# YHY138/Boosting-Fine-grained-Feature-Fusion-in-3D-Point-Cloud-Registration

Measured on AMD Instinct MI355X. Metric: point-cloud pairs/sec (forward) on ModelNet 2048-pt pairs, higher is better.
Workload: dtype f32 (emulated on the fp16 MFMA pipe: f16x3 split products); 1 GPU; ModelNet40 2048-pt pairs, 8 pairs per GPU (BASELINE configs[1] at N=1, configs[3] at N=8); pairs_per_gpu=8, global_batch=8, points_per_cloud=717, parallelism=pair-sharded dp1, precision=fp32

## Files before the change

boosting-fine-grained-feature-fusion-in-3d-point-cloud-registration_amd/csrc/ffn.hip:

```cpp
#include <algorithm>
#include <cstdlib>

#include "mfma.h"

namespace fgr {
namespace {

constexpr int kFfnD = 256;
constexpr int kFfnKS = kFfnD / 32;
constexpr int kFfnNP = kFfnD / 16;
constexpr int kFfnMaxF = 2048;
constexpr int kUnit = 1024;
constexpr int kRing = 8;
static_assert(kFfnKS * 128 == kUnit, "a W1 panel is one ring unit");
static_assert(kFfnNP / 2 * 128 == kUnit, "half of a chunk's W2 slice is one ring unit");

struct FfnArgs {
    const float* x; int64_t ldx;
    const float* ln_g; const float* ln_b; float eps;
    const u32x4* w1; const float* wsc1; const float* b1;
    const u32x4* w2; const float* wsc2; const float* b2;
    const float* bound;
    float* out; int64_t ldo;
    int M, F;
};

__device__ __forceinline__ void wait_units(int n) {
    static_assert(kRing - 2 <= 6, "extend the switch");
    switch (n) {
        case 0: wait_vm_lgkm0<0>(); break;
        case 1: wait_vm_lgkm0<4>(); break;
        case 2: wait_vm_lgkm0<8>(); break;
        case 3: wait_vm_lgkm0<12>(); break;
        case 4: wait_vm_lgkm0<16>(); break;
        case 5: wait_vm_lgkm0<20>(); break;
        default: wait_vm_lgkm0<24>(); break;
    }
}

typedef __attribute__((address_space(3))) u32x4 lds_u4;

__shared__ u32x4 g_ffn_ring0[kUnit], g_ffn_ring1[kUnit], g_ffn_ring2[kUnit], g_ffn_ring3[kUnit],
                 g_ffn_ring4[kUnit], g_ffn_ring5[kUnit], g_ffn_ring6[kUnit], g_ffn_ring7[kUnit];
static_assert(kRing == 8, "one object per slot below");

__device__ __forceinline__ u32x4* ring_slot(int s) {
    switch (s & 7) {
// ... 261 lines not shown
}

__device__ __forceinline__ float gelu_scaled(float sz, float isq) {
    const float a = sz * isq, t = fabsf(a), s = a * a;
    float r = fmaf(-1.72853470e-5f, t, 3.83197126e-4f);
    const float u = fmaf(-3.88396438e-3f, t, 2.42546219e-2f);
    r = fmaf(r, s, u);
    r = fmaf(r, t, -1.06777877e-1f);
    r = fmaf(r, t, -6.34846687e-1f);
    r = fmaf(r, t, -1.28717512e-1f);
    r = fmaf(r, t, -t);
    const float e = 0.5f * __expf(r);
    const float tail = a < 0.f ? e : 1.f - e;
    float q = -5.96761703e-4f;
    q = fmaf(q, s, 4.99119423e-3f);
    q = fmaf(q, s, -2.67681349e-2f);
    q = fmaf(q, s, 1.12819925e-1f);
    q = fmaf(q, s, -3.76125336e-1f);
    q = fmaf(q, s, 1.28379166e-1f);
    const float mid = fmaf(0.5f, fmaf(q, a, a), 0.5f);
    return sz * (t > 0.927734375f ? tail : mid);
}

template <int RT, int ACT = FGR_ACT_RELU>
__global__ void __launch_bounds__(256, 1) ffn_nsplit_kernel(FfnArgs p) {
    static_assert(RT >= 1 && RT <= 4, "row tiles");
    static_assert(ACT == FGR_ACT_RELU || ACT == FGR_ACT_GELU, "activation");
    __shared__ u32x4 act[RT * kFfnKS * 2 * 64];
    __shared__ u32x4 hbuf[2][4][RT][2][64];
    __shared__ float4 cw1[kFfnMaxF / 4], cb1[kFfnMaxF / 4];
    __shared__ float4 cw2[kFfnD / 4], cb2[kFfnD / 4];
    __shared__ float4 lng[kFfnD / 4], lnb[kFfnD / 4];
    __shared__ float2 rowpar[64];

    constexpr int BR = 16 * RT;
    const int nbm = (p.M + BR - 1) / BR;
    int t = blockIdx.x;
    {
        const int q = nbm / 8, r = nbm % 8, x = t % 8, lo = t / 8;
        t = (x < r ? x * (q + 1) : r * (q + 1) + (x - r) * q) + lo;
    }
    const int tid = threadIdx.x, wv = tid >> 6, lane = tid & 63;
    const int g = lane >> 4, c = lane & 15;
    const int r0 = t * BR;
    const int nst = p.F / 128;

    const int nf4 = p.F / 4;
    const int j0 = min(tid, nf4 - 1), j1 = min(tid + 256, nf4 - 1);
    const float4 pw1a = reinterpret_cast<const float4*>(p.wsc1)[j0];
    const float4 pb1a = reinterpret_cast<const float4*>(p.b1)[j0];
    const float4 pw1b = reinterpret_cast<const float4*>(p.wsc1)[j1];
    const float4 pb1b = reinterpret_cast<const float4*>(p.b1)[j1];
    const int t4 = tid & (kFfnD / 4 - 1);
    const float4 pw2 = reinterpret_cast<const float4*>(p.wsc2)[t4];
    const float4 pb2 = reinterpret_cast<const float4*>(p.b2)[t4];
    const float4 pg = reinterpret_cast<const float4*>(p.ln_g)[t4];
    const float4 pbe = reinterpret_cast<const float4*>(p.ln_b)[t4];
    __builtin_amdgcn_sched_barrier(0);
    float xr[kFfnKS][8];
    {
        const int64_t row = min(r0 + 16 * min(wv, RT - 1) + c, p.M - 1);
        const float* ar = p.x + row * p.ldx;
#pragma unroll
        for (int s = 0; s < kFfnKS; ++s) {
            const float4 a0 = *reinterpret_cast<const float4*>(ar + 32 * s + 8 * g);
            const float4 a1 = *reinterpret_cast<const float4*>(ar + 32 * s + 8 * g + 4);
            xr[s][0] = a0.x; xr[s][1] = a0.y; xr[s][2] = a0.z; xr[s][3] = a0.w;
            xr[s][4] = a1.x; xr[s][5] = a1.y; xr[s][6] = a1.z; xr[s][7] = a1.w;
        }
    }
    {
        if (tid < nf4) { cw1[tid] = pw1a; cb1[tid] = pb1a; }
        if (tid + 256 < nf4) { cw1[tid + 256] = pw1b; cb1[tid + 256] = pb1b; }
        if (tid < kFfnD / 4) { cw2[tid] = pw2; cb2[tid] = pb2; lng[tid] = pg; lnb[tid] = pbe; }
    }
    const float bM1 = p.bound[0], bMb = p.bound[1];
    __syncthreads();

    {
        float sm = 0.f;
#pragma unroll
        for (int s = 0; s < kFfnKS; ++s)
            sm += ((xr[s][0] + xr[s][1]) + (xr[s][2] + xr[s][3])) +
                  ((xr[s][4] + xr[s][5]) + (xr[s][6] + xr[s][7]));
        const float mean = xg_sum(sm) / (float)kFfnD;
        float sq = 0.f;
#pragma unroll
        for (int s = 0; s < kFfnKS; ++s)
#pragma unroll
            for (int e = 0; e < 8; ++e) {
                const float d = xr[s][e] - mean;
                sq += d * d;
            }
        const float rstd = 1.0f / sqrtf(xg_sum(sq) / (float)kFfnD + p.eps);
        float mx = 0.f, nn = 0.f;
#pragma unroll
        for (int s = 0; s < kFfnKS; ++s) {
            const int k = 32 * s + 8 * g;
            const float4 g0 = lng[k / 4], g1 = lng[k / 4 + 1];
            const float4 b0 = lnb[k / 4], b1 = lnb[k / 4 + 1];
            const float gg[8] = {g0.x, g0.y, g0.z, g0.w, g1.x, g1.y, g1.z, g1.w};
            const float bb[8] = {b0.x, b0.y, b0.z, b0.w, b1.x, b1.y, b1.z, b1.w};
// ... 150 lines not shown
                        const f16x8 wh = __builtin_bit_cast(f16x8, wf[2 * qq]);
                        const f16x8 wl = __builtin_bit_cast(f16x8, wf[2 * qq + 1]);
                        f32x4& a = accy[rt][2 * qh + qq];
                        a = __builtin_amdgcn_mfma_f32_16x16x32_f16(wl, hh, a, 0, 0, 0);
                        a = __builtin_amdgcn_mfma_f32_16x16x32_f16(wh, hl, a, 0, 0, 0);
                        a = __builtin_amdgcn_mfma_f32_16x16x32_f16(wh, hh, a, 0, 0, 0);
                    }
                }
                __builtin_amdgcn_sched_group_barrier(0x008, 6 * RT, 0);
                __builtin_amdgcn_sched_barrier(0);
            }
        }
    }
    wait_vm_only(0);

#pragma unroll
    for (int rt = 0; rt < RT; ++rt) {
        const int rr = r0 + 16 * rt + c;
        const int64_t row = min(rr, p.M - 1);
        const float inv_s = 1.f / rowpar[16 * rt + c].y;
        const float* xrow = p.x + row * p.ldx;
        float4 res[4];
#pragma unroll
        for (int q = 0; q < 4; ++q) res[q] = *reinterpret_cast<const float4*>(xrow + 16 * (4 * wv + q) + 4 * g);
        float* orow = p.out + row * p.ldo;
#pragma unroll
        for (int q = 0; q < 4; ++q) {
            const int n = 16 * (4 * wv + q) + 4 * g;
            const float4 w4 = cw2[n / 4], b4 = cb2[n / 4];
            const float4 y = make_float4(fmaf(accy[rt][q][0], w4.x * inv_s, b4.x) + res[q].x,
                                         fmaf(accy[rt][q][1], w4.y * inv_s, b4.y) + res[q].y,
                                         fmaf(accy[rt][q][2], w4.z * inv_s, b4.z) + res[q].z,
                                         fmaf(accy[rt][q][3], w4.w * inv_s, b4.w) + res[q].w);
            if (rr < p.M) *reinterpret_cast<float4*>(orow + n) = y;
        }
    }
}

__global__ void __launch_bounds__(256)
ffn_w2_split_kernel(const float* __restrict__ w, int n, int f, int64_t sn, int64_t sk,
                    float* __restrict__ wsc, u32x4* __restrict__ img) {
    const int tid = threadIdx.x, q = blockIdx.x, r0 = q * 16;
    const int ri = tid >> 4, kl = tid & 15;
    float mx = 0.f;
    if (r0 + ri < n)
        for (int j = kl; j < f; j += 16) mx = fmaxf(mx, fabsf(w[(int64_t)(r0 + ri) * sn + (int64_t)j * sk]));
    __shared__ float red[16][17];
    __shared__ float scale_inv[16];
    red[ri][kl] = mx;
    __syncthreads();
    if (tid < 16) {
        float m = 0.f;
#pragma unroll
        for (int z = 0; z < 16; ++z) m = fmaxf(m, red[tid][z]);
        const int e = row_scale_exp(m);
        const bool ok = r0 + tid < n;
        scale_inv[tid] = ok ? __builtin_ldexpf(1.f, e) : 0.f;
// ... 86 lines not shown
    if (m == 0) return FGR_OK;
    hipStream_t st = as_stream(stream);
    TimedCall timed_(st);
    const char* i1 = static_cast<const char*>(w1_img);
    const char* i2 = static_cast<const char*>(w2_img);
    FfnArgs a{x, ldx, gamma, beta, eps,
              (const u32x4*)i1, (const float*)(i1 + (size_t)(f / 16) * kFfnKS * 128 * 16), b1,
              (const u32x4*)i2, (const float*)(i2 + ffn_image_bytes(d, f)), b2,
              bound, out, ldo, m, f};
    const bool rt3 = (m + 47) / 48 <= kCusFfn && (m + 63) / 64 < kCusFfn;
    if (act == FGR_ACT_GELU) {
        const unsigned nb = (unsigned)((m + 47) / 48);
        hipLaunchKernelGGL((ffn_nsplit_kernel<3, FGR_ACT_GELU>), dim3(nb), dim3(256), 0, st, a);
    } else if (f % 128 == 0) {
        if (rt3)
            hipLaunchKernelGGL(ffn_nsplit_kernel<3>, dim3((unsigned)((m + 47) / 48)), dim3(256), 0, st, a);
        else
            hipLaunchKernelGGL(ffn_nsplit_kernel<4>, dim3((unsigned)((m + 63) / 64)), dim3(256), 0, st, a);
    } else
        hipLaunchKernelGGL(ffn_f16x3_kernel, dim3((unsigned)((m + 63) / 64)), dim3(256), 0, st, a);
    FGR_CHECK_LAUNCH("ffn_f16x3_kernel");
    return FGR_OK;
}
```

boosting-fine-grained-feature-fusion-in-3d-point-cloud-registration_amd/fgreg/_lib.py:

```python
import ctypes
import os
import subprocess

HERE = os.path.dirname(os.path.abspath(__file__))
LIB_PATH = os.environ.get('FGREG_LIB_PATH') or os.path.join(HERE, 'libfgreg.so')
CSRC = os.path.join(os.path.dirname(HERE), 'csrc')

_vp = ctypes.c_void_p
_i32 = ctypes.c_int32
_i64 = ctypes.c_int64
_f32 = ctypes.c_float
_sz = ctypes.c_size_t

ABI_VERSION = 2

SIGNATURES = {
    'fgr_grid_subsample_workspace': [_i64, _i32, _i64, ctypes.POINTER(_sz)],
    'fgr_grid_subsample_count': [_vp, _vp, _i32, _i64, _f32, _i64, _vp, _sz, _vp, _vp],
    'fgr_grid_subsample_fill': [_i64, _i32, _i64, _i64, _vp, _sz, _vp, _vp, _vp, _vp],
    'fgr_grid_subsample_sparse_workspace': [_i64, _i32, ctypes.POINTER(_sz)],
    'fgr_grid_subsample_sparse_count': [_vp, _vp, _i32, _i64, _f32, _i32, _vp, _sz, _vp, _vp],
    'fgr_grid_subsample_sparse_fill': [_i64, _i32, _i64, _vp, _sz, _vp, _vp, _vp, _vp],
    'fgr_radius_grid_workspace': [_i64, _i32, ctypes.POINTER(_sz)],
    'fgr_radius_grid_build': [_vp, _vp, _i32, _i64, _f32, _vp, _sz, _vp],
# ... 36 lines not shown
                                  ctypes.c_uint32, _f32, _vp, _vp],
    'fgr_attention_bf16_workspace': [_i64, _i32, _i32, ctypes.POINTER(_sz)],
    'fgr_attention_bf16': [_vp, _i64, _vp, _i64, _vp, _i64, _vp, _i64, _vp, _vp, _vp, _i32, _i32,
                           _i64, _i32, _i32, _i32, _i32, _f32, _vp, _i64, _vp],
    'fgr_res2net_chain6': [_vp, _i64, _i32, _i32, _vp, _vp, _vp, _i32, _vp, _i64, _vp],
    'fgr_res2net_chain_h3': [_vp, _i64, _i32, _i32, _vp, _vp, _vp, _vp, _i32, _vp, _i64, _vp],
    'fgr_res2net_block_h3': [_vp, _i64, _i32, _i32, _i32, _vp, _vp, _vp, _vp, _vp, _vp, _vp, _i64,
                             _vp],
    'fgr_res2net_block6': [_vp, _i64, _i32, _i32, _i32, _vp, _vp, _vp, _vp, _vp, _vp, _i64, _vp],
    'fgr_split_weights_h3_bytes': [_i32, _i32, ctypes.POINTER(_sz)],
    'fgr_split_weights_h3_batch': [_vp, _i32, _i64, _vp],
    'fgr_split_weights_h3': [_vp, _i32, _i32, _i64, _i64, _vp, _vp],
    'fgr_gemm_f16x3': [_vp, _i64, _vp, _vp, _i64, _vp, _vp, _i64, _i32, _i32, _i32, _i32, _vp],
    'fgr_gemm_f16x3_ln_supported': [_i32, _i32, _i32],
    'fgr_gemm_f16x3_ln': [_vp, _i64, _vp, _vp, _f32, _vp, _i64, _vp, _vp, _i64, _vp, _i32, _i32,
                          _i32, _i32, _vp],
    'fgr_gemm_f16x3_ln_out2': [_vp, _i64, _vp, _vp, _f32, _vp, _i64, _vp, _vp, _i64, _vp, _i32,
                               _i32, _i32, _i32, _vp, _vp, _vp, _i64, _vp],
    'fgr_split_weights_ffn2_bytes': [_i32, _i32, ctypes.POINTER(_sz)],
    'fgr_split_weights_ffn2': [_vp, _i32, _i32, _i64, _i64, _vp, _vp],
    'fgr_ffn_f16x3_supported': [_i32, _i32, _i32],
    'fgr_ffn_f16x3': [_vp, _i64, _vp, _vp, _f32, _vp, _vp, _vp, _vp, _vp, _vp, _i64, _i32, _i32,
                      _i32, _vp],
    'fgr_ffn_f16x3_act_supported': [_i32, _i32, _i32, _i32],
    'fgr_ffn_f16x3_act': [_vp, _i64, _vp, _vp, _f32, _vp, _vp, _vp, _vp, _vp, _vp, _i64, _i32,
                          _i32, _i32, _i32, _vp],
    'fgr_gelu_fwd': [_vp, _vp, _i64, _vp],
    'fgr_gelu_bwd': [_vp, _vp, _vp, _i64, _vp],
    'fgr_pos_mlp_f16x3_supported': [_i64, _i32],
    'fgr_pos_mlp_f16x3': [_vp, _i64, _vp, _vp, _vp, _vp, _vp, _vp, _vp, _vp, _vp, _vp, _i32, _vp,
                          _i64, _vp],
    'fgr_split_weights_bf16_bytes': [_i32, _i32, ctypes.POINTER(_sz)],
    'fgr_split_weights_bf16': [_vp, _i32, _i32, _i64, _i64, _vp, _vp],
    'fgr_gemm_bf16': [_vp, _i64, _vp, _vp, _i64, _vp, _vp, _i64, _i32, _i32, _i32, _i32, _vp],
    'fgr_gemm_workspace': [_i32, _i32, _i32, _i32, ctypes.POINTER(_sz)],
    'fgr_gemm_f16x3_ws': [_vp, _i64, _vp, _vp, _i64, _vp, _vp, _i64, _i32, _i32, _i32, _i32, _vp,
                          _sz, _vp],
    'fgr_gemm_bf16_ws': [_vp, _i64, _vp, _vp, _i64, _vp, _vp, _i64, _i32, _i32, _i32, _i32, _vp,
                         _sz, _vp],
    'fgr_kv_image_bytes': [_i64, _i32, _i32, ctypes.POINTER(_sz)],
    'fgr_gemm_f16x3_ln_qkv_supported': [_i32, _i32, _i32],
    'fgr_gemm_f16x3_ln_qkv': [_vp, _i64, _vp, _vp, _f32, _vp, _i64, _vp, _vp, _i64, _vp, _i32, _i32,
                              _i32, _vp, _vp, _vp, _vp, _i64, _vp],
    'fgr_gemm_f16x3_qkv_supported': [_i32, _i32, _i32],
    'fgr_gemm_f16x3_qkv': [_vp, _i64, _vp, _vp, _i64, _vp, _i32, _i32, _i32, _vp, _vp],
    'fgr_kv_image_bf16_bytes': [_i64, _i32, _i32, ctypes.POINTER(_sz)],
# ... 135 lines not shown
```

boosting-fine-grained-feature-fusion-in-3d-point-cloud-registration_amd/fgreg/ops.py:

```python
import ctypes
import math
from typing import Optional, Sequence, Tuple

import torch

from . import _lib
from ._lib import (ACT_GELU, ACT_LEAKY, ACT_NONE, ACT_RELU, ACT_RELU_RES_LEAKY,
                   NB_DIST, NB_INDEX)


def _ptr(t):
    return None if t is None else t.data_ptr()


class KernelTimer:

    def __init__(self, names):
        self.names = set(names)
        self.events = {n: [] for n in names}
        self.work = {n: [] for n in names}
        self.labels = {n: [] for n in names}
        self.count = False
        self.pool = []
        self.lead_cycles = 0
# ... 818 lines not shown
    t0 = _begin('gemm', (n, 3 * d, d))
    gemm_fn = 'fgr_gemm_f16x3_qkv' if mode == 'f16x3' else 'fgr_gemm_bf16_qkv'
    _lib.check(getattr(L, gemm_fn)(_ptr(h), h.stride(0), _ptr(w_img.img), _ptr(q), q.stride(0),
                                   _ptr(bias), n, d, n_head, _ptr(img), _stream()), gemm_fn)
    _end('gemm', t0, 2 * n * 3 * d * d)
    o = torch.empty((n, d), dtype=torch.float32, device=h.device)
    t0 = _begin('attention')
    attn_fn = 'fgr_attention_f16x3_img' if mode == 'f16x3' else 'fgr_attention_bf16_img'
    _lib.check(getattr(L, attn_fn)(
        _ptr(q), q.stride(0), _ptr(img), n, _ptr(o), o.stride(0), _ptr(q_off), _ptr(q_off),
        _ptr(kv_seg), q_off.numel() - 1, int(max_len), n_head, d // n_head,
        float(math.sqrt(1.0 / float(d // n_head))), _stream()), attn_fn)
    _end('attention', t0, lambda: attention_flops(q_off, q_off, kv_seg, d))
    return o


FFN_FUSE = True


def ffn_supported(m, d, f, act=ACT_RELU) -> bool:
    return FFN_FUSE and bool(_lib.load().fgr_ffn_f16x3_act_supported(m, d, f, act))


def ffn(x, norm, w1_img, b1, w2_img, b2, bound, out=None, act=ACT_RELU) -> torch.Tensor:
    _dev(x, b1, b2, bound)
    m, d = x.shape
    f = b1.numel()
    assert x.dtype == torch.float32 and x.stride(1) == 1 and b2.numel() == d
    x = x if (x.stride(0) % 4 == 0 and x.data_ptr() % 16 == 0) else x.contiguous()
    g, b = norm.weight.contiguous(), norm.bias.contiguous()
    b1, b2, bound = b1.contiguous(), b2.contiguous(), bound.contiguous()
    if out is None:
        out = torch.empty((m, d), dtype=torch.float32, device=x.device)
    t0 = _begin('gemm', ('ffn', m, d, f))
    _lib.check(_lib.load().fgr_ffn_f16x3_act(
        _ptr(x), x.stride(0), _ptr(g), _ptr(b), float(norm.eps), _ptr(w1_img.img), _ptr(b1),
        _ptr(w2_img.img), _ptr(b2), _ptr(bound), _ptr(out), out.stride(0), m, d, f, int(act),
        _stream()), 'fgr_ffn_f16x3_act')
    _end('gemm', t0, 4 * m * d * f)
    return out


def gelu(z, out=None) -> torch.Tensor:
    _dev(z, out)
    assert z.dtype == torch.float32 and z.is_contiguous()
    if out is None:
        out = torch.empty_like(z)
    assert out.dtype == torch.float32 and out.is_contiguous() and out.shape == z.shape
    _lib.check(_lib.load().fgr_gelu_fwd(_ptr(z), _ptr(out), z.numel(), _stream()), 'fgr_gelu_fwd')
    return out


def gelu_(z) -> torch.Tensor:
    return gelu(z, out=z)


def gelu_backward(z, dy, out=None) -> torch.Tensor:
    _dev(z, dy, out)
    assert z.dtype == torch.float32 and z.is_contiguous()
    dy = _c(dy, torch.float32)
    assert dy.shape == z.shape
    if out is None:
# ... 119 lines not shown
```

boosting-fine-grained-feature-fusion-in-3d-point-cloud-registration_amd/fgreg/transformer.py:

```python
import copy

import torch
import torch.nn as nn

from . import linear as lin
from . import ops
from .linear import linear, linear_ln, ln_fusable

class Segments:

    def __init__(self, lengths, device, n_layers=0, phantoms=None):
        self.lengths = [int(n) for n in lengths]
        n = len(self.lengths)
        assert n % 2 == 0
        self.B = n // 2
        self.phantoms = [int(p) for p in phantoms] if phantoms is not None else [0] * n
        assert len(self.phantoms) == n and min(self.phantoms, default=0) >= 0
        self.seg_cloud = list(range(n)) + [c for c in range(n) if self.phantoms[c] > 0]
        self.seg_lengths = self.lengths + [p for p in self.phantoms if p > 0]
        self.n_phantom = sum(self.phantoms)
        self.off = ops.offsets(self.seg_lengths, device)
        self.cloud_off = self.off[:n + 1]
        self.self_seg = ops.to_device(self.seg_cloud, torch.int32, device)
        self.cross_seg = ops.to_device([(c + self.B) % n for c in self.seg_cloud], torch.int32,
# ... 66 lines not shown
                and ops.qkv_bf16_supported(h_pos.shape[0], d, self.nhead)):
            return ops.qkv_attention(h_pos, lin.weight_image(W, mode='bf16'), b, seg.off, kv_seg,
                                     seg.max_len, self.nhead, mode='bf16')
        if val_has_pos:
            qkv = linear(h_pos, W, b)
            q, k, v = qkv[:, :d], qkv[:, d:2 * d], qkv[:, 2 * d:]
        else:
            qk = linear(h_pos, W, b[:2 * d], rows=(0, 2 * d))
            q, k = qk[:, :d], qk[:, d:]
            v = linear(h_nopos, W, b[2 * d:], rows=(2 * d, 3 * d))
        o = ops.attention(q, k, v, seg.off, seg.off, kv_seg, seg.max_len, self.nhead)
        return o

    def takes_side(self, x, pos):
        n, d = x.shape
        return (self.normalize_before and self.sa_val_has_pos_emb and pos is not None
                and ln_fusable(n, 3 * d, d))

    def wants_h1(self, x):
        n, d = x.shape
        return (self.normalize_before and self.sa_val_has_pos_emb
                and not ln_fusable(n, 3 * d, d))

    def forward_packed(self, x, pos, seg: Segments, pending_bias=None, h1=None, side=None):
        if not self.normalize_before:
            return self._forward_post(x, pos, seg, pending_bias), None
        n, d = x.shape
        fuse_in = ln_fusable(n, 3 * d, d)
        if fuse_in and self.sa_val_has_pos_emb and pending_bias is None:
            o = self._attend(self.self_attn, None, None, True, seg, seg.self_seg,
                             ln=(x, self.norm1, pos), side=side)
            side = None
        elif h1 is not None:
            assert pending_bias is None and self.sa_val_has_pos_emb
            o = self._attend(self.self_attn, h1, None, True, seg, seg.self_seg)
        else:
            if side is not None:
                ops.layernorm(x, side[0].weight, side[0].bias, side[0].eps, out=side[1])
                side = None
            h = ops.layernorm(x, self.norm1.weight, self.norm1.bias, self.norm1.eps, add=pos,
                              pre_bias=pending_bias)
            h0 = None if self.sa_val_has_pos_emb else ops.layernorm(
                x, self.norm1.weight, self.norm1.bias, self.norm1.eps)
            o = self._attend(self.self_attn, h, h0, self.sa_val_has_pos_emb, seg, seg.self_seg)
        x = linear(o, self.self_attn.out_proj.weight, self.self_attn.out_proj.bias, residual=x)
        if fuse_in and self.ca_val_has_pos_emb:
            o = self._attend(self.multihead_attn, None, None, True, seg, seg.cross_seg,
                             ln=(x, self.norm2, pos))
        else:
            h = ops.layernorm(x, self.norm2.weight, self.norm2.bias, self.norm2.eps, add=pos)
            h0 = None if self.ca_val_has_pos_emb else ops.layernorm(
                x, self.norm2.weight, self.norm2.bias, self.norm2.eps)
            o = self._attend(self.multihead_attn, h, h0, self.ca_val_has_pos_emb, seg,
                             seg.cross_seg)
        x = linear(o, self.multihead_attn.out_proj.weight, self.multihead_attn.out_proj.bias,
                   residual=x)
        if lin.MODE == 'f16x3' and ops.ffn_supported(n, d, self.linear1.out_features, self.act):
            return ops.ffn(x, self.norm3, lin.weight_image(self.linear1.weight, mode='f16x3'),
                           self.linear1.bias, lin.weight_image(self.linear2.weight, mode='ffn2'),
                           self.linear2.bias, self._ffn_bound(), act=self.act), None
        if self.act == ops.ACT_GELU:
            h = ops.gelu_(linear_ln(x, self.norm3, self.linear1.weight, self.linear1.bias))
        else:
            h = linear_ln(x, self.norm3, self.linear1.weight, self.linear1.bias, act=ops.ACT_RELU)
        return linear(h, self.linear2.weight, self.linear2.bias, residual=x), None

    def _ffn_bound(self):
        w, b = self.linear1.weight, self.linear1.bias
        key = (w.data_ptr(), w._version, b.data_ptr(), b._version)
        st = self.__dict__.get('_ffn_bound_cache')
        if st is None or st[0] != key:
            with torch.no_grad():
                bound = torch.stack([w.detach().norm(dim=1).max(),
                                     b.detach().abs().max()]).float().contiguous()
            st = (key, bound)
            self.__dict__['_ffn_bound_cache'] = st
            ops.note_state(bound)
# ... 16 lines not shown
            h = linear(x, self.linear1.weight, self.linear1.bias, act=ops.ACT_RELU)
        t = linear(h, self.linear2.weight, self.linear2.bias, residual=x)
        return ops.layernorm(t, self.norm3.weight, self.norm3.bias, self.norm3.eps)


class TransformerCrossEncoder(nn.Module):

    def __init__(self, cross_encoder_layer, num_layers, norm=None, return_intermediate=False):
        super().__init__()
        self.layers = nn.ModuleList([copy.deepcopy(cross_encoder_layer) for _ in range(num_layers)])
        self.num_layers = num_layers
        self.norm = norm
        self.return_intermediate = return_intermediate

    def forward_packed(self, x, pos, seg: Segments):
        L = len(self.layers)
        n, d = x.shape
        inter = torch.empty((L if self.return_intermediate else 1, n, d), dtype=x.dtype,
                            device=x.device)
        x = x.clone()
        pending = None
        h1 = side = None
        for l, layer in enumerate(self.layers):
            x, pending = layer.forward_packed(x, pos, seg, pending, h1=h1, side=side)
            h1 = side = None
            if self.return_intermediate or l == L - 1:
                nxt = self.layers[l + 1] if l + 1 < L else None
                if (nxt is not None and self.norm is not None and pending is None
                        and nxt.takes_side(x, pos) and self.norm.eps == nxt.norm1.eps):
                    side = (self.norm, inter[l if self.return_intermediate else 0])
                elif (nxt is not None and self.norm is not None and pending is None
                        and nxt.wants_h1(x) and self.norm.eps == nxt.norm1.eps):
                    _, h1 = ops.layernorm_dual(x, self.norm, nxt.norm1, add_b=pos,
                                               out_a=inter[l if self.return_intermediate else 0])
                else:
                    self._norm(x, pending, inter[l if self.return_intermediate else 0])
                pending = None
        return inter

    def _norm(self, x, pending, out):
        if self.norm is None:
            if pending is not None:
                x.add_(pending)
            out.copy_(x)
            return out
        return ops.layernorm(x, self.norm.weight, self.norm.bias, self.norm.eps,
                             pre_bias=pending, out=out)

# ... 56 lines not shown
```

include/fgreg.h:

```cpp
#ifndef FGREG_H
#define FGREG_H

#include <stddef.h>
#include <stdint.h>

#ifdef __cplusplus
extern "C" {
#endif

#define FGR_ABI_VERSION 2

enum {
    FGR_OK = 0,
    FGR_E_ARG = -1,
    FGR_E_LAUNCH = -2,
    FGR_E_WORKSPACE = -3
};

enum {
    FGR_NB_INDEX = 0,
    FGR_NB_DIST = 1
};

enum { FGR_ACT_NONE = 0, FGR_ACT_LEAKY = 1, FGR_ACT_RELU = 2, FGR_ACT_RELU_RES_LEAKY = 3,
// ... 148 lines not shown
int fgr_gemm_f16x3_ln(const float* x, int64_t ldx, const float* gamma, const float* beta,
                      float eps, const float* add, int64_t ld_add, const void* w_img, float* c,
                      int64_t ldc, const float* bias, int32_t m, int32_t n, int32_t k,
                      int32_t act, void* stream);
int fgr_gemm_f16x3_ln_out2(const float* x, int64_t ldx, const float* gamma, const float* beta,
                           float eps, const float* add, int64_t ld_add, const void* w_img,
                           float* c, int64_t ldc, const float* bias, int32_t m, int32_t n,
                           int32_t k, int32_t act, const float* gamma2, const float* beta2,
                           float* out2, int64_t ld_out2, void* stream);

int fgr_split_weights_ffn2_bytes(int32_t n, int32_t k, size_t* bytes);
int fgr_split_weights_ffn2(const float* w, int32_t n, int32_t k, int64_t stride_n,
                           int64_t stride_k, void* img, void* stream);
int fgr_ffn_f16x3_supported(int32_t m, int32_t d, int32_t f);
int fgr_ffn_f16x3(const float* x, int64_t ldx, const float* gamma, const float* beta, float eps,
                  const void* w1_img, const float* b1, const void* w2_img, const float* b2,
                  const float* bound, float* out, int64_t ldo, int32_t m, int32_t d, int32_t f,
                  void* stream);
int fgr_ffn_f16x3_act_supported(int32_t m, int32_t d, int32_t f, int32_t act);
int fgr_ffn_f16x3_act(const float* x, int64_t ldx, const float* gamma, const float* beta,
                      float eps, const void* w1_img, const float* b1, const void* w2_img,
                      const float* b2, const float* bound, float* out, int64_t ldo, int32_t m,
                      int32_t d, int32_t f, int32_t act, void* stream);

int fgr_pos_mlp_f16x3_supported(int64_t n, int32_t d_model);
int fgr_pos_mlp_f16x3(const float* xyz, int64_t n, const float* w0, const float* b0,
                      const void* w1_img, const float* b1, const void* w2_img, const float* b2,
                      const void* w3_img, const float* b3, const void* w4_img, const float* b4,
                      int32_t d_model, float* out, int64_t ldo, void* stream);

int fgr_split_weights_bf16_bytes(int32_t n, int32_t k, size_t* bytes);
int fgr_split_weights_bf16(const float* w, int32_t n, int32_t k, int64_t stride_n,
                           int64_t stride_k, void* img, void* stream);
int fgr_gemm_bf16(const float* a, int64_t lda, const void* w_img, float* c, int64_t ldc,
                  const float* bias, const float* r, int64_t ldr, int32_t m, int32_t n, int32_t k,
                  int32_t act, void* stream);

int fgr_attention(const float* q, int64_t ld_q, const float* k, int64_t ld_k, const float* v,
                  int64_t ld_v, float* o, int64_t ld_o, const int64_t* q_off,
                  const int64_t* kv_off, const int32_t* kv_seg, int32_t n_seg,
                  int32_t max_q_len, int32_t n_head, int32_t head_dim, float scale, void* stream);

int fgr_attention_f16x3_workspace(int64_t n_kv_rows, int32_t n_kv_seg, int32_t n_head,
                                  size_t* bytes);
int fgr_attention_f16x3(const float* q, int64_t ld_q, const float* k, int64_t ld_k,
                        const float* v, int64_t ld_v, float* o, int64_t ld_o,
// ... 226 lines not shown
```

Measured before the change: 3267 pairs/s.

## Fuse attention out-projection and final LayerNorm into the fused FFN kernel

Adds a TAIL variant of the fused FFN kernel that first computes the cross-attention output projection (f16x3 MFMA) plus residual, then runs LayerNorm and the FFN within the same block. For the last layer it can also apply the decoder's final LayerNorm and write that second output directly. This removes a separate linear launch, a norm launch, and the global round-trip of the intermediate activations. In exchange the kernel uses more LDS and registers and adds several block-wide reductions and syncs, which could lower occupancy or lengthen the prologue.

```diff
diff --git a/boosting-fine-grained-feature-fusion-in-3d-point-cloud-registration_amd/csrc/ffn.hip b/boosting-fine-grained-feature-fusion-in-3d-point-cloud-registration_amd/csrc/ffn.hip
--- a/boosting-fine-grained-feature-fusion-in-3d-point-cloud-registration_amd/csrc/ffn.hip
+++ b/boosting-fine-grained-feature-fusion-in-3d-point-cloud-registration_amd/csrc/ffn.hip
@@ -23,6 +23,9 @@
     const float* bound;
     float* out; int64_t ldo;
     int M, F;
+    const float* o; int64_t ldao;
+    const u32x4* wo; const float* wsco; const float* bo;
+    float* out2; int64_t ld2; const float* g2; const float* be2; float eps2;
 };
 
 __device__ __forceinline__ void wait_units(int n) {
@@ -330,10 +333,14 @@
     return sz * (t > 0.927734375f ? tail : mid);
 }
 
-template <int RT, int ACT = FGR_ACT_RELU>
+template <int RT, int ACT = FGR_ACT_RELU, bool TAIL = false>
 __global__ void __launch_bounds__(256, 1) ffn_nsplit_kernel(FfnArgs p) {
     static_assert(RT >= 1 && RT <= 4, "row tiles");
     static_assert(ACT == FGR_ACT_RELU || ACT == FGR_ACT_GELU, "activation");
+    __shared__ float4 cwo[TAIL ? kFfnD / 4 : 1], cbo[TAIL ? kFfnD / 4 : 1];
+    __shared__ float osc[TAIL ? 64 : 1];
+    __shared__ float red0[4][TAIL ? 64 : 1], red1[4][TAIL ? 64 : 1];
+    __shared__ float2 red2[4][TAIL ? 64 : 1];
     __shared__ u32x4 act[RT * kFfnKS * 2 * 64];
     __shared__ u32x4 hbuf[2][4][RT][2][64];
     __shared__ float4 cw1[kFfnMaxF / 4], cb1[kFfnMaxF / 4];
@@ -364,11 +371,16 @@
     const float4 pb2 = reinterpret_cast<const float4*>(p.b2)[t4];
     const float4 pg = reinterpret_cast<const float4*>(p.ln_g)[t4];
     const float4 pbe = reinterpret_cast<const float4*>(p.ln_b)[t4];
+    float4 pwo, pbo;
+    if constexpr (TAIL) {
+        pwo = reinterpret_cast<const float4*>(p.wsco)[t4];
+        pbo = reinterpret_cast<const float4*>(p.bo)[t4];
+    }
     __builtin_amdgcn_sched_barrier(0);
     float xr[kFfnKS][8];
     {
         const int64_t row = min(r0 + 16 * min(wv, RT - 1) + c, p.M - 1);
-        const float* ar = p.x + row * p.ldx;
+        const float* ar = TAIL ? p.o + row * p.ldao : p.x + row * p.ldx;
 #pragma unroll
         for (int s = 0; s < kFfnKS; ++s) {
             const float4 a0 = *reinterpret_cast<const float4*>(ar + 32 * s + 8 * g);
@@ -383,9 +395,180 @@
         if (tid < kFfnD / 4) { cw2[tid] = pw2; cb2[tid] = pb2; lng[tid] = pg; lnb[tid] = pbe; }
     }
     const float bM1 = p.bound[0], bMb = p.bound[1];
-    __syncthreads();
-
-    {
+
+    float xp[TAIL ? RT : 1][4][4];
+    if constexpr (TAIL) {
+        u32x4 wr[3][8];
+        auto issue0 = [&](int s, u32x4 (&slot)[8]) {
+#pragma unroll
+            for (int e = 0; e < 8; ++e)
+                slot[e] = p.wo[(((int64_t)(4 * wv + (e >> 1)) * kFfnKS + s) * 2 + (e & 1)) * 64 + lane];
+        };
+        issue0(0, wr[0]);
+        issue0(1, wr[1]);
+#pragma unroll
+        for (int rt = 0; rt < RT; ++rt) {
+            const float* xrow = p.x + (int64_t)min(r0 + 16 * rt + c, p.M - 1) * p.ldx;
+#pragma unroll
+            for (int q = 0; q < 4; ++q) {
+                const float4 v = ld4(xrow + 16 * (4 * wv + q) + 4 * g);
+                xp[rt][q][0] = v.x; xp[rt][q][1] = v.y; xp[rt][q][2] = v.z; xp[rt][q][3] = v.w;
+            }
+        }
+        __builtin_amdgcn_sched_barrier(0);
+        if (tid < kFfnD / 4) { cwo[tid] = pwo; cbo[tid] = pbo; }
+        {
+            float mx = 0.f;
+#pragma unroll
+            for (int s = 0; s < kFfnKS; ++s) {
+                mx = fmaxf(mx, max3_abs(xr[s][0], xr[s][1], xr[s][2]));
+                mx = fmaxf(mx, max3_abs(xr[s][3], xr[s][4], xr[s][5]));
+                mx = fmaxf(mx, max3_abs(xr[s][6], xr[s][7], 0.f));
+            }
+            const int eo = row_scale_exp(xg_max(mx));
+            const float sco = __builtin_ldexpf(1.f, eo);
+            if (wv < RT) {
+#pragma unroll
+                for (int s = 0; s < kFfnKS; ++s) {
+                    u32x4 h, l;
+                    split8_f16(xr[s], sco, h, l);
+                    act[((wv * kFfnKS + s) * 2 + 0) * 64 + lane] = h;
+                    act[((wv * kFfnKS + s) * 2 + 1) * 64 + lane] = l;
+                }
+                if (g == 0) osc[16 * wv + c] = __builtin_ldexpf(1.f, -eo);
+            }
+        }
+        __syncthreads();
+        f32x4 a0[RT][4];
+#pragma unroll
+        for (int rt = 0; rt < RT; ++rt)
+#pragma unroll
+            for (int q = 0; q < 4; ++q) a0[rt][q] = f32x4{0.f, 0.f, 0.f, 0.f};
+        u32x4 fo[2][2 * RT];
+        auto read_o = [&](int s, u32x4 (&f)[2 * RT]) {
+#pragma unroll
+            for (int rt = 0; rt < RT; ++rt) {
+                f[2 * rt + 0] = act[((rt * kFfnKS + s) * 2 + 0) * 64 + lane];
+                f[2 * rt + 1] = act[((rt * kFfnKS + s) * 2 + 1) * 64 + lane];
+            }
+        };
+        read_o(0, fo[0]);
+#pragma unroll
+        for (int s = 0; s < kFfnKS; ++s) {
+            if (s + 2 < kFfnKS) issue0(s + 2, wr[(s + 2) % 3]);
+            if (s + 1 < kFfnKS) read_o(s + 1, fo[(s + 1) & 1]);
+            u32x4 (&wf)[8] = wr[s % 3];
+            u32x4 (&cur)[2 * RT] = fo[s & 1];
+#pragma unroll
+            for (int rt = 0; rt < RT; ++rt) {
+                const f16x8 ah = __builtin_bit_cast(f16x8, cur[2 * rt + 0]);
+                const f16x8 al = __builtin_bit_cast(f16x8, cur[2 * rt + 1]);
+#pragma unroll
+                for (int q = 0; q < 4; ++q) {
+                    const f16x8 wh = __builtin_bit_cast(f16x8, wf[2 * q]);
+                    const f16x8 wl = __builtin_bit_cast(f16x8, wf[2 * q + 1]);
+                    a0[rt][q] = __builtin_amdgcn_mfma_f32_16x16x32_f16(wl, ah, a0[rt][q], 0, 0, 0);
+                    a0[rt][q] = __builtin_amdgcn_mfma_f32_16x16x32_f16(wh, al, a0[rt][q], 0, 0, 0);
+                    a0[rt][q] = __builtin_amdgcn_mfma_f32_16x16x32_f16(wh, ah, a0[rt][q], 0, 0, 0);
+                }
+            }
+        }
+#pragma unroll
+        for (int rt = 0; rt < RT; ++rt) {
+            const float is = osc[16 * rt + c];
+            float sm = 0.f;
+#pragma unroll
+            for (int q = 0; q < 4; ++q) {
+                const int n = 16 * (4 * wv + q) + 4 * g;
+                const float4 w4 = cwo[n / 4], b4 = cbo[n / 4];
+                xp[rt][q][0] = fmaf(a0[rt][q][0], w4.x * is, b4.x) + xp[rt][q][0];
+                xp[rt][q][1] = fmaf(a0[rt][q][1], w4.y * is, b4.y) + xp[rt][q][1];
+                xp[rt][q][2] = fmaf(a0[rt][q][2], w4.z * is, b4.z) + xp[rt][q][2];
+                xp[rt][q][3] = fmaf(a0[rt][q][3], w4.w * is, b4.w) + xp[rt][q][3];
+                sm += (xp[rt][q][0] + xp[rt][q][1]) + (xp[rt][q][2] + xp[rt][q][3]);
+            }
+            sm = xg_sum(sm);
+            if (g == 0) red0[wv][16 * rt + c] = sm;
+        }
+        __syncthreads();
+        float mean[RT];
+#pragma unroll
+        for (int rt = 0; rt < RT; ++rt) {
+            const int r = 16 * rt + c;
+            mean[rt] = (((red0[0][r] + red0[1][r]) + red0[2][r]) + red0[3][r]) / (float)kFfnD;
+            float sq = 0.f;
+#pragma unroll
+            for (int q = 0; q < 4; ++q)
+#pragma unroll
+                for (int e = 0; e < 4; ++e) {
+                    const float d = xp[rt][q][e] - mean[rt];
+                    sq = fmaf(d, d, sq);
+                }
+            sq = xg_sum(sq);
+            if (g == 0) red1[wv][r] = sq;
+        }
+        __syncthreads();
+        float an[RT][4][4];
+#pragma unroll
+        for (int rt = 0; rt < RT; ++rt) {
+            const int r = 16 * rt + c;
+            const float var = (((red1[0][r] + red1[1][r]) + red1[2][r]) + red1[3][r]) / (float)kFfnD;
+            const float rstd = 1.0f / sqrtf(var + p.eps);
+            float mx = 0.f, nn = 0.f;
+#pragma unroll
+            for (int q = 0; q < 4; ++q) {
+                const int n = 16 * (4 * wv + q) + 4 * g;
+                const float4 g4 = lng[n / 4], b4 = lnb[n / 4];
+                const float gg[4] = {g4.x, g4.y, g4.z, g4.w}, bb[4] = {b4.x, b4.y, b4.z, b4.w};
+#pragma unroll
+                for (int e = 0; e < 4; ++e) {
+                    const float a = (xp[rt][q][e] - mean[rt]) * rstd * gg[e] + bb[e];
+                    an[rt][q][e] = a;
+                    nn = fmaf(a, a, nn);
+                }
+                mx = fmaxf(mx, max3_abs(an[rt][q][0], an[rt][q][1], an[rt][q][2]));
+                mx = fmaxf(mx, fabsf(an[rt][q][3]));
+            }
+            mx = xg_max(mx);
+            nn = xg_sum(nn);
+            if (g == 0) red2[wv][r] = make_float2(mx, nn);
+        }
+        __syncthreads();
+#pragma unroll
+        for (int rt = 0; rt < RT; ++rt) {
+            const int r = 16 * rt + c;
+            const float2 t0 = red2[0][r], t1 = red2[1][r], t2 = red2[2][r], t3 = red2[3][r];
+            const float mx = fmaxf(fmaxf(t0.x, t1.x), fmaxf(t2.x, t3.x));
+            const float nn = ((t0.y + t1.y) + t2.y) + t3.y;
+            const int ea = row_scale_exp(mx);
+            const float sca = __builtin_ldexpf(1.f, ea);
+#pragma unroll
+            for (int q = 0; q < 4; ++q) {
+                const int qp = 4 * wv + q;
+                _Float16 h[4], l[4];
+#pragma unroll
+                for (int e = 0; e < 4; ++e) {
+                    const float v = an[rt][q][e] * sca;
+                    h[e] = (_Float16)v;
+                    l[e] = (_Float16)(v - (float)h[e]);
+                }
+                typedef _Float16 f16x4 __attribute__((ext_vector_type(4)));
+                const f16x4 hv = {h[0], h[1], h[2], h[3]}, lv = {l[0], l[1], l[2], l[3]};
+                const int u = ((rt * kFfnKS + (qp >> 1)) * 2) * 64 + (2 * (qp & 1) + (g >> 1)) * 16 + c;
+                f16x4* dst = reinterpret_cast<f16x4*>(act) + (g & 1);
+                dst[2 * u] = hv;
+                dst[2 * (u + 64)] = lv;
+            }
+            const float bnd = sqrtf(nn) * bM1 + bMb;
+            const int eh = bnd > 0.f ? max(min(15 - __builtin_amdgcn_frexp_expf(bnd), 127), -126) : 0;
+            if (wv == 0 && g == 0)
+                rowpar[r] = make_float2(__builtin_ldexpf(1.f, eh - ea), __builtin_ldexpf(1.f, eh));
+        }
+    } else {
+        __syncthreads();
+    }
+
+    if constexpr (!TAIL) {
         float sm = 0.f;
 #pragma unroll
         for (int s = 0; s < kFfnKS; ++s)
@@ -582,7 +765,10 @@
         const float* xrow = p.x + row * p.ldx;
         float4 res[4];
 #pragma unroll
-        for (int q = 0; q < 4; ++q) res[q] = *reinterpret_cast<const float4*>(xrow + 16 * (4 * wv + q) + 4 * g);
+        for (int q = 0; q < 4; ++q) {
+            if constexpr (TAIL) res[q] = make_float4(xp[rt][q][0], xp[rt][q][1], xp[rt][q][2], xp[rt][q][3]);
+            else res[q] = *reinterpret_cast<const float4*>(xrow + 16 * (4 * wv + q) + 4 * g);
+        }
         float* orow = p.out + row * p.ldo;
 #pragma unroll
         for (int q = 0; q < 4; ++q) {
@@ -593,6 +779,54 @@
                                          fmaf(accy[rt][q][2], w4.z * inv_s, b4.z) + res[q].z,
                                          fmaf(accy[rt][q][3], w4.w * inv_s, b4.w) + res[q].w);
             if (rr < p.M) *reinterpret_cast<float4*>(orow + n) = y;
+            if constexpr (TAIL) accy[rt][q] = f32x4{y.x, y.y, y.z, y.w};
+        }
+    }
+    if constexpr (TAIL) {
+        if (p.out2 == nullptr) return;
+#pragma unroll
+        for (int rt = 0; rt < RT; ++rt) {
+            float sm = 0.f;
+#pragma unroll
+            for (int q = 0; q < 4; ++q)
+                sm += (accy[rt][q][0] + accy[rt][q][1]) + (accy[rt][q][2] + accy[rt][q][3]);
+            sm = xg_sum(sm);
+            if (g == 0) red0[wv][16 * rt + c] = sm;
+        }
+        __syncthreads();
+        float mean[RT];
+#pragma unroll
+        for (int rt = 0; rt < RT; ++rt) {
+            const int r = 16 * rt + c;
+            mean[rt] = (((red0[0][r] + red0[1][r]) + red0[2][r]) + red0[3][r]) / (float)kFfnD;
+            float sq = 0.f;
+#pragma unroll
+            for (int q = 0; q < 4; ++q)
+#pragma unroll
+                for (int e = 0; e < 4; ++e) {
+                    const float d = accy[rt][q][e] - mean[rt];
+                    sq = fmaf(d, d, sq);
+                }
+            sq = xg_sum(sq);
+            if (g == 0) red1[wv][r] = sq;
+        }
+        __syncthreads();
+#pragma unroll
+        for (int rt = 0; rt < RT; ++rt) {
+            const int r = 16 * rt + c, rr = r0 + r;
+            const float var = (((red1[0][r] + red1[1][r]) + red1[2][r]) + red1[3][r]) / (float)kFfnD;
+            const float rstd = 1.0f / sqrtf(var + p.eps2);
+            float* orow = p.out2 + (int64_t)min(rr, p.M - 1) * p.ld2;
+#pragma unroll
+            for (int q = 0; q < 4; ++q) {
+                const int n = 16 * (4 * wv + q) + 4 * g;
+                const float4 g4 = ld4(p.g2 + n), b4 = ld4(p.be2 + n);
+                const float4 y = make_float4((accy[rt][q][0] - mean[rt]) * rstd * g4.x + b4.x,
+                                             (accy[rt][q][1] - mean[rt]) * rstd * g4.y + b4.y,
+                                             (accy[rt][q][2] - mean[rt]) * rstd * g4.z + b4.z,
+                                             (accy[rt][q][3] - mean[rt]) * rstd * g4.w + b4.w);
+                if (rr < p.M) *reinterpret_cast<float4*>(orow + n) = y;
+            }
         }
     }
 }
@@ -725,3 +959,70 @@
     FGR_CHECK_LAUNCH("ffn_f16x3_kernel");
     return FGR_OK;
 }
+
+extern "C" int fgr_attn_out_ffn_f16x3_supported(int32_t m, int32_t d, int32_t f, int32_t n_head,
+                                                int32_t act) {
+    return (fgr_ffn_f16x3_act_supported(m, d, f, act) && f % 128 == 0 && n_head > 0 &&
+            n_head * 32 == d) ? 1 : 0;
+}
+
+extern "C" int fgr_attn_out_ffn_f16x3(const float* o, int64_t ld_o, const void* wo_img,
+                                      const float* bo, const float* x, int64_t ldx,
+                                      const float* gamma, const float* beta, float eps,
+                                      const void* w1_img, const float* b1, const void* w2_img,
+                                      const float* b2, const float* bound, float* out, int64_t ldo,
+                                      const float* gamma2, const float* beta2, float eps2,
+                                      float* out2, int64_t ld_out2, int32_t m, int32_t d,
+                                      int32_t f, int32_t n_head, int32_t act, void* stream) {
+    FGR_REQUIRE(o && wo_img && bo && x && gamma && beta && w1_img && b1 && w2_img && b2 && bound &&
+                    out && m >= 0 && ld_o >= d && ldx >= d && ldo >= d && eps >= 0.f,
+                "fgr_attn_out_ffn_f16x3: bad arguments");
+    FGR_REQUIRE(!out2 || (gamma2 && beta2 && ld_out2 >= d && eps2 >= 0.f),
+                "fgr_attn_out_ffn_f16x3: out2 needs gamma2, beta2 and ld_out2 >= d");
+    FGR_REQUIRE(m == 0 || fgr_attn_out_ffn_f16x3_supported(m, d, f, n_head, act),
+                "fgr_attn_out_ffn_f16x3: d %d, hidden %d, heads %d, act %d not supported "
+                "(fgr_attn_out_ffn_f16x3_supported)", d, f, n_head, act);
+    const uintptr_t al = reinterpret_cast<uintptr_t>(o) | reinterpret_cast<uintptr_t>(wo_img) |
+                         reinterpret_cast<uintptr_t>(bo) | reinterpret_cast<uintptr_t>(x) |
+                         reinterpret_cast<uintptr_t>(gamma) | reinterpret_cast<uintptr_t>(beta) |
+                         reinterpret_cast<uintptr_t>(w1_img) | reinterpret_cast<uintptr_t>(b1) |
+                         reinterpret_cast<uintptr_t>(w2_img) | reinterpret_cast<uintptr_t>(b2) |
+                         reinterpret_cast<uintptr_t>(out) | reinterpret_cast<uintptr_t>(out2) |
+                         reinterpret_cast<uintptr_t>(gamma2) | reinterpret_cast<uintptr_t>(beta2);
+    FGR_REQUIRE((al & 15) == 0 && ld_o % 4 == 0 && ldx % 4 == 0 && ldo % 4 == 0 &&
+                    (!out2 || ld_out2 % 4 == 0),
+                "fgr_attn_out_ffn_f16x3: operands must be 16-B aligned with row strides %% 4 == 0");
+    auto apart = [m](const float* a, int64_t lda, const float* b, int64_t ldb) {
+        return a + (size_t)m * lda <= b || b + (size_t)m * ldb <= a;
+    };
+    FGR_REQUIRE(out == x || apart(out, ldo, x, ldx),
+                "fgr_attn_out_ffn_f16x3: out overlaps x partially");
+    FGR_REQUIRE(apart(out, ldo, o, ld_o), "fgr_attn_out_ffn_f16x3: out overlaps o");
+    FGR_REQUIRE(!out2 || (apart(out2, ld_out2, o, ld_o) && apart(out2, ld_out2, x, ldx) &&
+                          apart(out2, ld_out2, out, ldo)),
+                "fgr_attn_out_ffn_f16x3: out2 overlaps o, x or out");
+    if (m == 0) return FGR_OK;
+    hipStream_t st = as_stream(stream);
+    TimedCall timed_(st);
+    const char* i0 = static_cast<const char*>(wo_img);
+    const char* i1 = static_cast<const char*>(w1_img);
+    const char* i2 = static_cast<const char*>(w2_img);
+    FfnArgs a{x, ldx, gamma, beta, eps,
+              (const u32x4*)i1, (const float*)(i1 + (size_t)(f / 16) * kFfnKS * 128 * 16), b1,
+              (const u32x4*)i2, (const float*)(i2 + ffn_image_bytes(d, f)), b2,
+              bound, out, ldo, m, f,
+              o, ld_o, (const u32x4*)i0, (const float*)(i0 + (size_t)kFfnNP * kFfnKS * 128 * 16), bo,
+              out2, ld_out2, gamma2, beta2, eps2};
+    const bool rt3 = (m + 47) / 48 <= kCusFfn && (m + 63) / 64 < kCusFfn;
+    if (act == FGR_ACT_GELU)
+        hipLaunchKernelGGL((ffn_nsplit_kernel<3, FGR_ACT_GELU, true>),
+                           dim3((unsigned)((m + 47) / 48)), dim3(256), 0, st, a);
+    else if (rt3)
+        hipLaunchKernelGGL((ffn_nsplit_kernel<3, FGR_ACT_RELU, true>),
+                           dim3((unsigned)((m + 47) / 48)), dim3(256), 0, st, a);
+    else
+        hipLaunchKernelGGL((ffn_nsplit_kernel<4, FGR_ACT_RELU, true>),
+                           dim3((unsigned)((m + 63) / 64)), dim3(256), 0, st, a);
+    FGR_CHECK_LAUNCH("ffn_nsplit_kernel (attention tail)");
+    return FGR_OK;
+}
diff --git a/boosting-fine-grained-feature-fusion-in-3d-point-cloud-registration_amd/fgreg/_lib.py b/boosting-fine-grained-feature-fusion-in-3d-point-cloud-registration_amd/fgreg/_lib.py
--- a/boosting-fine-grained-feature-fusion-in-3d-point-cloud-registration_amd/fgreg/_lib.py
+++ b/boosting-fine-grained-feature-fusion-in-3d-point-cloud-registration_amd/fgreg/_lib.py
@@ -82,6 +82,10 @@
     'fgr_ffn_f16x3_supported': [_i32, _i32, _i32],
     'fgr_ffn_f16x3': [_vp, _i64, _vp, _vp, _f32, _vp, _vp, _vp, _vp, _vp, _vp, _i64, _i32, _i32,
                       _i32, _vp],
+    'fgr_attn_out_ffn_f16x3_supported': [_i32, _i32, _i32, _i32, _i32],
+    'fgr_attn_out_ffn_f16x3': [_vp, _i64, _vp, _vp, _vp, _i64, _vp, _vp, _f32, _vp, _vp, _vp, _vp,
+                               _vp, _vp, _i64, _vp, _vp, _f32, _vp, _i64, _i32, _i32, _i32, _i32,
+                               _i32, _vp],
     'fgr_ffn_f16x3_act_supported': [_i32, _i32, _i32, _i32],
     'fgr_ffn_f16x3_act': [_vp, _i64, _vp, _vp, _f32, _vp, _vp, _vp, _vp, _vp, _vp, _i64, _i32,
                           _i32, _i32, _i32, _vp],
diff --git a/boosting-fine-grained-feature-fusion-in-3d-point-cloud-registration_amd/fgreg/ops.py b/boosting-fine-grained-feature-fusion-in-3d-point-cloud-registration_amd/fgreg/ops.py
--- a/boosting-fine-grained-feature-fusion-in-3d-point-cloud-registration_amd/fgreg/ops.py
+++ b/boosting-fine-grained-feature-fusion-in-3d-point-cloud-registration_amd/fgreg/ops.py
@@ -864,7 +864,13 @@
     return FFN_FUSE and bool(_lib.load().fgr_ffn_f16x3_act_supported(m, d, f, act))
 
 
-def ffn(x, norm, w1_img, b1, w2_img, b2, bound, out=None, act=ACT_RELU) -> torch.Tensor:
+def ffn(x, norm, w1_img, b1, w2_img, b2, bound, out=None, act=ACT_RELU, tail=None, norm2=None,
+        out2=None) -> torch.Tensor:
+    if tail is not None:
+        o, wo_img, bo, n_head = tail
+        return attn_out_ffn(o, wo_img, bo, x, norm, w1_img, b1, w2_img, b2, bound, n_head,
+                            out=out, act=act, norm2=norm2, out2=out2)
+    assert out2 is None
     _dev(x, b1, b2, bound)
     m, d = x.shape
     f = b1.numel()
@@ -880,6 +886,46 @@
         _ptr(w2_img.img), _ptr(b2), _ptr(bound), _ptr(out), out.stride(0), m, d, f, int(act),
         _stream()), 'fgr_ffn_f16x3_act')
     _end('gemm', t0, 4 * m * d * f)
+    return out
+
+
+ATTN_OUT_FFN = True
+
+
+def attn_out_ffn_supported(m, d, f, n_head, act=ACT_RELU) -> bool:
+    return ATTN_OUT_FFN and FFN_FUSE and bool(
+        _lib.load().fgr_attn_out_ffn_f16x3_supported(m, d, f, n_head, act))
+
+
+def attn_out_ffn(o, wo_img, bo, x, norm, w1_img, b1, w2_img, b2, bound, n_head, out=None,
+                 act=ACT_RELU, norm2=None, out2=None) -> torch.Tensor:
+    _dev(o, x, bo, b1, b2, bound)
+    m, d = x.shape
+    f = b1.numel()
+    assert o.shape == x.shape and bo.numel() == d and b2.numel() == d
+    assert x.dtype == torch.float32 and x.stride(1) == 1 and o.dtype == torch.float32
+
+    def _rows(t):
+        return t if (t.stride(1) == 1 and t.stride(0) % 4 == 0 and t.data_ptr() % 16 == 0) \
+            else t.contiguous()
+    o, x = _rows(o), _rows(x)
+    g, b = norm.weight.contiguous(), norm.bias.contiguous()
+    bo, b1, b2, bound = bo.contiguous(), b1.contiguous(), b2.contiguous(), bound.contiguous()
+    if out is None:
+        out = torch.empty((m, d), dtype=torch.float32, device=x.device)
+    g2 = b2n = None
+    eps2, ld2 = 0.0, 0
+    if out2 is not None:
+        assert norm2 is not None and out2.shape == x.shape and out2.stride(1) == 1
+        g2, b2n, eps2, ld2 = norm2.weight.contiguous(), norm2.bias.contiguous(), norm2.eps, \
+            out2.stride(0)
+    t0 = _begin('gemm', ('ffn', m, d, f))
+    _lib.check(_lib.load().fgr_attn_out_ffn_f16x3(
+        _ptr(o), o.stride(0), _ptr(wo_img.img), _ptr(bo), _ptr(x), x.stride(0), _ptr(g), _ptr(b),
+        float(norm.eps), _ptr(w1_img.img), _ptr(b1), _ptr(w2_img.img), _ptr(b2), _ptr(bound),
+        _ptr(out), out.stride(0), _ptr(g2), _ptr(b2n), float(eps2), _ptr(out2), ld2, m, d, f,
+        int(n_head), int(act), _stream()), 'fgr_attn_out_ffn_f16x3')
+    _end('gemm', t0, 4 * m * d * f + 2 * m * d * d)
     return out
 
 
diff --git a/boosting-fine-grained-feature-fusion-in-3d-point-cloud-registration_amd/fgreg/transformer.py b/boosting-fine-grained-feature-fusion-in-3d-point-cloud-registration_amd/fgreg/transformer.py
--- a/boosting-fine-grained-feature-fusion-in-3d-point-cloud-registration_amd/fgreg/transformer.py
+++ b/boosting-fine-grained-feature-fusion-in-3d-point-cloud-registration_amd/fgreg/transformer.py
@@ -112,7 +112,16 @@
         return (self.normalize_before and self.sa_val_has_pos_emb
                 and not ln_fusable(n, 3 * d, d))
 
-    def forward_packed(self, x, pos, seg: Segments, pending_bias=None, h1=None, side=None):
+    def _tail_ffn(self, n, d):
+        return (self.normalize_before and lin.MODE == 'f16x3'
+                and ops.attn_out_ffn_supported(n, d, self.linear1.out_features, self.nhead,
+                                               self.act))
+
+    def takes_out2(self, x):
+        return self._tail_ffn(*x.shape)
+
+    def forward_packed(self, x, pos, seg: Segments, pending_bias=None, h1=None, side=None,
+                       out2=None):
         if not self.normalize_before:
             return self._forward_post(x, pos, seg, pending_bias), None
         n, d = x.shape
@@ -143,6 +152,16 @@
                 x, self.norm2.weight, self.norm2.bias, self.norm2.eps)
             o = self._attend(self.multihead_attn, h, h0, self.ca_val_has_pos_emb, seg,
                              seg.cross_seg)
+        if self._tail_ffn(n, d):
+            op = self.multihead_attn.out_proj
+            return ops.ffn(
+                x, self.norm3, lin.weight_image(self.linear1.weight, mode='f16x3'),
+                self.linear1.bias, lin.weight_image(self.linear2.weight, mode='ffn2'),
+                self.linear2.bias, self._ffn_bound(), act=self.act,
+                tail=(o, lin.weight_image(op.weight, mode='f16x3'), op.bias, self.nhead),
+                norm2=out2[0] if out2 is not None else None,
+                out2=out2[1] if out2 is not None else None), None
+        assert out2 is None
         x = linear(o, self.multihead_attn.out_proj.weight, self.multihead_attn.out_proj.bias,
                    residual=x)
         if lin.MODE == 'f16x3' and ops.ffn_supported(n, d, self.linear1.out_features, self.act):
@@ -205,8 +224,14 @@
         pending = None
         h1 = side = None
         for l, layer in enumerate(self.layers):
-            x, pending = layer.forward_packed(x, pos, seg, pending, h1=h1, side=side)
+            out2 = None
+            if l == L - 1 and self.norm is not None and layer.takes_out2(x):
+                out2 = (self.norm, inter[l if self.return_intermediate else 0])
+            x, pending = layer.forward_packed(x, pos, seg, pending, h1=h1, side=side, out2=out2)
             h1 = side = None
+            if out2 is not None:
+                assert pending is None
+                continue
             if self.return_intermediate or l == L - 1:
                 nxt = self.layers[l + 1] if l + 1 < L else None
                 if (nxt is not None and self.norm is not None and pending is None
diff --git a/include/fgreg.h b/include/fgreg.h
--- a/include/fgreg.h
+++ b/include/fgreg.h
@@ -194,6 +194,15 @@
                       float eps, const void* w1_img, const float* b1, const void* w2_img,
                       const float* b2, const float* bound, float* out, int64_t ldo, int32_t m,
                       int32_t d, int32_t f, int32_t act, void* stream);
+int fgr_attn_out_ffn_f16x3_supported(int32_t m, int32_t d, int32_t f, int32_t n_head,
+                                     int32_t act);
+int fgr_attn_out_ffn_f16x3(const float* o, int64_t ld_o, const void* wo_img, const float* bo,
+                           const float* x, int64_t ldx, const float* gamma, const float* beta,
+                           float eps, const void* w1_img, const float* b1, const void* w2_img,
+                           const float* b2, const float* bound, float* out, int64_t ldo,
+                           const float* gamma2, const float* beta2, float eps2, float* out2,
+                           int64_t ld_out2, int32_t m, int32_t d, int32_t f, int32_t n_head,
+                           int32_t act, void* stream);
 
 int fgr_pos_mlp_f16x3_supported(int64_t n, int32_t d_model);
 int fgr_pos_mlp_f16x3(const float* xyz, int64_t n, const float* w0, const float* b0,
```

Result: no change. 3278 pairs/s, median of 6 (+0.4%).
